# powei-lin/camera-intrinsic-calibration-rs

Measured on AMD Instinct MI355X. Metric: corner residual+Jacobian evals/sec; LM iters/sec to converge (EUCM, TUM-VI cam0), higher is better.
Workload: dtype f64

## Files before the change

camera_intrinsic_calibration_rs_amd/csrc/ccal_api.hip:

```cpp
#include <algorithm>
#include <cmath>
#include <cstdio>
#include <cstring>
#include <memory>
#include <new>

#include "ccal_call.hpp"
#include "ccal_normal.hpp"

using namespace ccal;

static void stream_synced(ccal_problem* p) {
    if (!p->nws) return;
    p->nws->tail_pending = false;
    if (p->nws->fws) p->nws->fws->tail_pending = false;
}

static void default_conventions(ccal_model_conventions* cv) {
    cv->kb4_small_radius = kDefaultKb4SmallRadius;
    cv->unproject_small_radius = kDefaultUnprojectSmallRadius;
    for (int i = 0; i < 5; ++i) cv->ocv5_order[i] = i;
    cv->reserved_ = 0;
    for (int m = 0; m < kNumModels; ++m)
        for (int i = 0; i < kMaxDist; ++i) { cv->dist_lo[m][i] = kDefaultDistLo[m][i]; cv->dist_hi[m][i] = kDefaultDistHi[m][i]; }
}
static_assert(sizeof(((ccal_model_conventions*)nullptr)->dist_lo) == sizeof(kDefaultDistLo), "conventions table shape");

extern "C" {

int ccal_get_model_conventions(const ccal_ctx* ctx, ccal_model_conventions* out) {
    if (!ctx || !out) return CCAL_ERR_INVALID_ARG;
    *out = ctx->conv;
    return CCAL_OK;
}
int ccal_set_model_conventions(ccal_ctx* ctx, const ccal_model_conventions* in) {
    if (!ctx) return CCAL_ERR_INVALID_ARG;
    if (!in) { default_conventions(&ctx->conv); return CCAL_OK; }
    if (!(in->kb4_small_radius >= 0.0) || !(in->unproject_small_radius >= 0.0)) return CCAL_ERR_INVALID_ARG;
    {
        int seen = 0;
        for (int i = 0; i < 5; ++i) { if (in->ocv5_order[i] < 0 || in->ocv5_order[i] > 4) return CCAL_ERR_INVALID_ARG; seen |= 1 << in->ocv5_order[i]; }
        if (seen != 31) return CCAL_ERR_INVALID_ARG;
    }
    for (int m = 0; m < kNumModels; ++m)
        for (int i = 0; i < model_np(m) - 4; ++i) if (!(in->dist_lo[m][i] <= in->dist_hi[m][i])) return CCAL_ERR_INVALID_ARG;
    ctx->conv = *in;
    return CCAL_OK;
}

const char* ccal_version(void) { return "ccal-mi355x 0.3.0 (gfx950)"; }
int ccal_model_num_params(int model) { return (model >= 0 && model < kNumModels) ? model_np(model) : model == CCAL_MODEL_EUCMT ? 8 : -1; }

int ccal_ctx_create(int device_id, void* hip_stream, ccal_ctx** out) {
    if (!out) return CCAL_ERR_INVALID_ARG;
    *out = nullptr;
    int n = 0;
    if (hipGetDeviceCount(&n) != hipSuccess || n <= 0) { (void)hipGetLastError(); note_create_error("ccal_ctx_create: no HIP device"); return CCAL_ERR_HIP; }
    if (device_id < 0 || device_id >= n) { note_create_error("ccal_ctx_create: device " + std::to_string(device_id) + " of " + std::to_string(n)); return CCAL_ERR_HIP; }
    ccal_ctx* c = new (std::nothrow) ccal_ctx();
    if (!c) return CCAL_ERR_NO_MEMORY;
    default_conventions(&c->conv);
    c->device = device_id;
    if (hipSetDevice(device_id) != hipSuccess) { delete c; note_create_error("ccal_ctx_create: hipSetDevice failed"); return CCAL_ERR_HIP; }
    if (hip_stream) { c->stream = (hipStream_t)hip_stream; c->own_stream = false; }
    else {
        if (hipStreamCreateWithFlags(&c->stream, hipStreamNonBlocking) != hipSuccess) { delete c; note_create_error("ccal_ctx_create: hipStreamCreate failed"); return CCAL_ERR_HIP; }
        c->own_stream = true;
    }
    *out = c;
    return CCAL_OK;
}
static void ctx_free(ccal_ctx* ctx) {
    ctx_worker_destroy(ctx);
    (void)hipSetDevice(ctx->device);
    ctx_release(ctx, ctx->d_batch_tab, false); ctx_release(ctx, ctx->h_batch_tab, true);
    ctx_cache_clear(ctx);
    if (!ctx->pinned.empty()) {
        (void)hipSetDevice(ctx->device);
        if (ctx->stream) (void)hipStreamSynchronize(ctx->stream);
        for (auto& pr : ctx->pinned) (void)hipHostUnregister(pr.first);
        (void)hipGetLastError();
        ctx->pinned.clear();
    }
    if (ctx->own_stream && ctx->stream) { (void)hipSetDevice(ctx->device); (void)hipStreamDestroy(ctx->stream); }
    delete ctx;
}
}
namespace ccal {
void ctx_unref(ccal_ctx* ctx) {
    if (--ctx->n_problems == 0 && ctx->destroy_requested) ctx_free(ctx);
}
}
extern "C" {
void ccal_ctx_destroy(ccal_ctx* ctx) {
    if (!ctx) return;
    if (ctx->n_problems > 0) { ctx->destroy_requested = true; return; }
    ctx_free(ctx);
}
const char* ccal_last_error(const ccal_ctx* ctx) { return ctx ? ctx->err.c_str() : "null context"; }
int ccal_sync(ccal_ctx* ctx) {
    if (!ctx) return CCAL_ERR_INVALID_ARG;
    HIP_TRY(ctx, hipSetDevice(ctx->device));
    HIP_TRY(ctx, hipStreamSynchronize(ctx->stream));
    return CCAL_OK;
}

int ccal_pin_buffer(ccal_ctx* ctx, void* host_ptr, size_t bytes) {
    if (!ctx || !host_ptr || !bytes) return CCAL_ERR_INVALID_ARG;
    CCAL_API_TRY
    HIP_TRY(ctx, hipSetDevice(ctx->device));
    for (auto& pr : ctx->pinned) if (pr.first == host_ptr) return fail(ctx, CCAL_ERR_INVALID_ARG, "ccal_pin_buffer: this address is pinned already");
    if (pinned_device_ptr(host_ptr, bytes)) return CCAL_OK;
    ctx->pinned.reserve(ctx->pinned.size() + 1);
    const hipError_t e = hipHostRegister(host_ptr, bytes, hipHostRegisterMapped | hipHostRegisterPortable);
    if (e != hipSuccess) { (void)hipGetLastError(); return fail(ctx, CCAL_ERR_HIP, (std::string("ccal_pin_buffer: hipHostRegister: ") + hipGetErrorString(e)).c_str()); }
    ctx->pinned.emplace_back(host_ptr, bytes);
    return CCAL_OK;
    CCAL_API_CATCH(ctx)
}
int ccal_unpin_buffer(ccal_ctx* ctx, void* host_ptr) {
    if (!ctx || !host_ptr) return CCAL_ERR_INVALID_ARG;
    CCAL_API_TRY
    for (size_t i = 0; i < ctx->pinned.size(); ++i) {
        if (ctx->pinned[i].first != host_ptr) continue;
        HIP_TRY(ctx, hipSetDevice(ctx->device));
        HIP_TRY(ctx, hipStreamSynchronize(ctx->stream));
        ctx->pinned.erase(ctx->pinned.begin() + (ptrdiff_t)i);
        HIP_TRY(ctx, hipHostUnregister(host_ptr));
        return CCAL_OK;
    }
    return CCAL_OK;
    CCAL_API_CATCH(ctx)
}

int ccal_set_defaults(ccal_solver_opts* o) {
    if (!o) return CCAL_ERR_INVALID_ARG;
    o->method = CCAL_METHOD_GN; o->max_iterations = 100;
    o->min_abs_error_decrease = 1e-5; o->min_rel_error_decrease = 1e-5; o->min_error = 1e-10;
    o->lm_initial_radius = 1e4; o->lm_min_diagonal = 1e-6; o->lm_max_diagonal = 1e32;
    o->verbose = 0; o->timeout_s = 0;
    o->error_metric = CCAL_ERROR_SQUARED_NORM; o->reserved_ = 0;
    return CCAL_OK;
}

int ccal_problem_create(ccal_ctx* ctx, const ccal_problem_desc* d, ccal_problem** out) {
    if (!ctx || !d || !out) return CCAL_ERR_INVALID_ARG;
    *out = nullptr;
    CCAL_API_TRY
    if (d->n_cams < 1 || d->n_cams > CCAL_MAX_CAMS || d->n_slots < 0 || d->n_obs < 0 || !d->model ||
        (d->n_obs > 0 && (!d->obs_cam || !d->obs_slot || !d->obs_offsets)))
        return fail(ctx, CCAL_ERR_INVALID_ARG, "bad problem description");
    HIP_TRY(ctx, hipSetDevice(ctx->device));
    struct Destroy { void operator()(ccal_problem* q) const { ccal_problem_destroy(q); } };
    std::unique_ptr<ccal_problem, Destroy> hold(new ccal_problem());
    ccal_problem* p = hold.get();
    p->ctx = ctx; p->n_cams = d->n_cams; p->n_slots = d->n_slots; p->n_obs = d->n_obs;
    p->one_focal = d->xy_same_focal != 0; p->huber_delta = d->huber_delta;
    p->cams.resize(d->n_cams);
    int K = 0;
    for (int c = 0; c < d->n_cams; ++c) {
        CamLayout& cl = p->cams[c];
        cl.model = d->model[c];
        if (cl.model == CCAL_MODEL_EUCMT) return fail(ctx, CCAL_ERR_UNSUPPORTED, "EUCMT is a parameter container in this build (its projection is only in the absent camera-intrinsic-model crate)");
        if (cl.model < 0 || cl.model >= kNumModels) return fail(ctx, CCAL_ERR_INVALID_ARG, "unknown camera model");
        cl.P = model_np(cl.model); cl.Peff = cl.P - (p->one_focal ? 1 : 0);
        cl.D = cl.Peff + (c == 0 ? 6 : 12);
        cl.col_theta = K; K += cl.Peff;
        if (c > 0) { cl.col_extr = K; K += 6; }
        cl.width = d->width ? d->width[c] : 0.0; cl.height = d->height ? d->height[c] : 0.0;
    }
    if (K >= CCAL_KMAX) return fail(ctx, CCAL_ERR_INVALID_ARG, "reduced system too large");
    p->K = K;
    if (d->n_obs > 0) {
        p->h_obs_off.assign(d->obs_offsets, d->obs_offsets + d->n_obs + 1);
        p->h_obs_cam.assign(d->obs_cam, d->obs_cam + d->n_obs);
        p->h_obs_slot.assign(d->obs_slot, d->obs_slot + d->n_obs);
    } else {
        p->h_obs_off.assign(1, 0);
    }
    p->h_joff.resize(d->n_obs + 1);
    std::vector<uint8_t> seen((size_t)d->n_cams * (size_t)std::max(d->n_slots, 1), 0);
    int64_t j = 0;
    for (int o = 0; o < d->n_obs; ++o) {
        const int cam = p->h_obs_cam[o], slot = p->h_obs_slot[o];
        const int64_t n = p->h_obs_off[o + 1] - p->h_obs_off[o];
        if (cam < 0 || cam >= d->n_cams || slot < 0 || slot >= d->n_slots || n < 0 || p->h_obs_off[0] != 0)
            return fail(ctx, CCAL_ERR_INVALID_ARG, "bad observation frame table");
        uint8_t& sn = seen[(size_t)cam * d->n_slots + slot];
        if (sn) return fail(ctx, CCAL_ERR_INVALID_ARG, "two observation frames for the same (camera, slot)");
        sn = 1;
        p->h_joff[o] = j; j += n * 2 * p->cams[cam].D;
        p->cams[cam].obs.push_back(o);
    }
    p->h_joff[d->n_obs] = j; p->j_len = j;
    p->slot_ident = d->n_slots == d->n_obs;
    for (int o = 0; o < d->n_obs && p->slot_ident; ++o) p->slot_ident = p->h_obs_slot[o] == o;
    p->n_corners = p->h_obs_off[d->n_obs];
    if (p->n_corners >= ((int64_t)1 << 30)) return fail(ctx, CCAL_ERR_INVALID_ARG, "more than 2^30 - 1 corners in one problem: shard the frames (ccal_multi_problem_create)");
    const size_t nc = (size_t)p->n_corners;
    if (nc && (!d->p3d_x || !d->p3d_y || !d->p3d_z || !d->p2d_u || !d->p2d_v)) return fail(ctx, CCAL_ERR_INVALID_ARG, "null corner arrays");
    {
        uint32_t any = 0;
        for (size_t i = 0; i < nc; ++i) { uint32_t b; std::memcpy(&b, d->p3d_z + i, sizeof b); any |= b & 0x7fffffffu; }
        p->has_nonplanar = any != 0;
    }
    std::vector<int32_t> bin_tab;
    if (d->n_cams == 1 && d->n_obs > 0) {
        std::vector<int32_t> order;
        const int m0 = p->cams[0].model;
        p->gram_bins = gram2_bin_plan(p->h_obs_off.data(), d->n_obs, m0 == kUCM || m0 == kEUCM, &order);
        if (p->gram_bins.n_bins > 0) {
            bin_tab.assign((size_t)d->n_obs * 4 + 4, 0);
            for (int i = 0; i < d->n_obs; ++i) {
                const int o = order[(size_t)i];
                bin_tab[4 * (size_t)i] = o; bin_tab[4 * (size_t)i + 1] = (int32_t)p->h_obs_off[o];
                bin_tab[4 * (size_t)i + 2] = (int32_t)(p->h_obs_off[o + 1] - p->h_obs_off[o]); bin_tab[4 * (size_t)i + 3] = p->h_obs_slot[o];
            }
        }
    }
    size_t cam_obs[CCAL_MAX_CAMS];
    for (int c = 0; c < d->n_cams; ++c) cam_obs[c] = p->cams[c].obs.size();
    const ProblemLayout l((size_t)p->n_corners, (size_t)d->n_obs, (size_t)d->n_slots, d->n_cams, cam_obs, bin_tab.size());
    const size_t total = l.plan.total;
    HIP_TRY(ctx, ctx_dev_alloc(ctx, (void**)&p->d_block, total));
    char* h_pack = nullptr;
    struct PackGuard { ccal_ctx* c; char*& p; ~PackGuard() { if (p) { (void)hipStreamSynchronize(c->stream); ccal::ctx_release(c, p, true); } } } pack_guard{ ctx, h_pack };
    if (total <= ((size_t)8 << 20)) HIP_TRY(ctx, ctx_host_alloc(ctx, (void**)&h_pack, total));
    if (!h_pack) HIP_TRY(ctx, hipMemsetAsync(p->d_block, 0, total, ctx->stream));
    {
        const Bound dev{ p->d_block }, img{ h_pack };
        auto put = [&](auto** dst, auto slice, const auto* src, size_t n) -> hipError_t {
            *dst = dev.at(slice);
            const size_t nb = src ? n * sizeof(*src) : 0;
            if (!h_pack) return nb ? hipMemcpyAsync(*dst, src, nb, hipMemcpyHostToDevice, ctx->stream) : hipSuccess;
            if (nb) std::memcpy(img.at(slice), src, nb);
            if (slice.bytes) std::memset((char*)img.at(slice) + nb, 0, slice.bytes - nb);
            return hipSuccess;
        };
        HIP_TRY(ctx, put(&p->d_x, l.x, d->p3d_x, nc)); HIP_TRY(ctx, put(&p->d_y, l.y, d->p3d_y, nc)); HIP_TRY(ctx, put(&p->d_z, l.z, d->p3d_z, nc));
        HIP_TRY(ctx, put(&p->d_u, l.u, d->p2d_u, nc)); HIP_TRY(ctx, put(&p->d_v, l.v, d->p2d_v, nc));
        HIP_TRY(ctx, put(&p->d_obs_off, l.obs_off, p->h_obs_off.data(), p->h_obs_off.size()));
        HIP_TRY(ctx, put(&p->d_joff, l.joff, p->h_joff.data(), p->h_joff.size()));
        HIP_TRY(ctx, put(&p->d_obs_cam, l.obs_cam, p->h_obs_cam.data(), p->h_obs_cam.size()));
        HIP_TRY(ctx, put(&p->d_obs_slot, l.obs_slot, p->h_obs_slot.data(), p->h_obs_slot.size()));
        for (int c = 0; c < d->n_cams; ++c) HIP_TRY(ctx, put(&p->cams[c].d_obs, l.cam_obs[c], p->cams[c].obs.data(), p->cams[c].obs.size()));
        HIP_TRY(ctx, put(&p->d_bin_tab, l.bin_tab, bin_tab.data(), bin_tab.size()));
        p->d_intr = dev.at(l.intr); p->d_poses = dev.at(l.poses); p->d_extr = dev.at(l.extr);
        p->d_intr_c = dev.at(l.intr_c); p->d_poses_c = dev.at(l.poses_c); p->d_extr_c = dev.at(l.extr_c);
        if (h_pack) {
            HIP_TRY(ctx, hipMemcpyAsync(p->d_block, h_pack, l.uploaded, hipMemcpyHostToDevice, ctx->stream));
            HIP_TRY(ctx, hipMemsetAsync(p->d_block + l.uploaded, 0, total - l.uploaded, ctx->stream));
        }
    }
    const size_t ni = (size_t)d->n_cams * CCAL_PMAX;
    p->lo.assign(ni, 0.0); p->hi.assign(ni, 0.0); p->has_bound.assign(ni, 0); p->fixed.assign(ni, 0);
    if (hipStreamSynchronize(ctx->stream) != hipSuccess) return fail(ctx, CCAL_ERR_HIP, "upload failed");
    p->counted = true;
    ctx->n_problems += 1;
    *out = hold.release();
    return CCAL_OK;
    CCAL_API_CATCH(ctx)
}

void ccal_problem_destroy(ccal_problem* p) {
    if (!p) return;
    if (p->nws && p->ctx && (p->nws->tail_pending || (p->nws->fws && p->nws->fws->tail_pending))) {
        (void)hipSetDevice(p->ctx->device);
        (void)hipDeviceSynchronize();
        p->nws->tail_pending = false;
        if (p->nws->fws) p->nws->fws->tail_pending = false;
    }
    ccal_ctx* ctx = p->ctx;
    if (ctx && (p->d_block || p->nws)) {
        (void)hipSetDevice(ctx->device);
        if (ctx->own_stream && ctx->stream) (void)hipStreamSynchronize(ctx->stream); else (void)hipDeviceSynchronize();
        (void)hipGetLastError();
    }
    void* ptrs[] = { p->d_block, p->d_r, p->d_J, p->d_err, p->d_scratch };
    for (void* q : ptrs) if (q) ctx_release(ctx, q, false);
    normal_ws_destroy(p);
    const bool counted = p->counted;
    delete p;
    if (ctx && counted && --ctx->n_problems == 0 && ctx->destroy_requested) ctx_free(ctx);
}

int64_t ccal_num_corners(const ccal_problem* p) { return p ? p->n_corners : -1; }
int ccal_reduced_dim(const ccal_problem* p) { return p ? p->K : -1; }
int ccal_block_dim(const ccal_problem* p, int cam) { return (p && cam >= 0 && cam < p->n_cams) ? p->cams[cam].D : -1; }
int ccal_eff_num_params(const ccal_problem* p, int cam) { return (p && cam >= 0 && cam < p->n_cams) ? p->cams[cam].Peff : -1; }
int64_t ccal_jacobian_len(const ccal_problem* p) { return p ? p->j_len : -1; }

static bool idx_ok(const ccal_problem* p, int cam, int idx) {
    return p && cam >= 0 && cam < p->n_cams && idx >= 0 && idx < p->cams[cam].Peff;
}
int ccal_set_bounds(ccal_problem* p, int cam, int idx, double lo, double hi) {
    if (!idx_ok(p, cam, idx) || !(lo <= hi)) return CCAL_ERR_INVALID_ARG;
    p->lo[cam * CCAL_PMAX + idx] = lo; p->hi[cam * CCAL_PMAX + idx] = hi; p->has_bound[cam * CCAL_PMAX + idx] = 1;
    return CCAL_OK;
}
int ccal_clear_bounds(ccal_problem* p, int cam, int idx) {
    if (!idx_ok(p, cam, idx)) return CCAL_ERR_INVALID_ARG;
    p->has_bound[cam * CCAL_PMAX + idx] = 0; return CCAL_OK;
}
int ccal_fix_param(ccal_problem* p, int cam, int idx) {
    if (!idx_ok(p, cam, idx)) return CCAL_ERR_INVALID_ARG;
    p->fixed[cam * CCAL_PMAX + idx] = 1; return CCAL_OK;
}
int ccal_unfix_param(ccal_problem* p, int cam, int idx) {
    if (!idx_ok(p, cam, idx)) return CCAL_ERR_INVALID_ARG;
    p->fixed[cam * CCAL_PMAX + idx] = 0; return CCAL_OK;
}

int ccal_apply_reference_bounds(ccal_problem* p) {
    if (!p) return CCAL_ERR_INVALID_ARG;
    const int shift = p->one_focal ? 1 : 0;
    const ccal_model_conventions& cv = p->ctx->conv;
    for (int c = 0; c < p->n_cams; ++c) {
        const CamLayout& cl = p->cams[c];
        ccal_set_bounds(p, c, 0, 0.0, 10000.0);
        ccal_set_bounds(p, c, 1 - shift, 0.0, 10000.0);
        ccal_set_bounds(p, c, 2 - shift, 0.0, cl.width);
        ccal_set_bounds(p, c, 3 - shift, 0.0, cl.height);
        for (int i = 4; i < cl.P; ++i) {
            const int at = cl.model == kOCV5 ? 4 + cv.ocv5_order[i - 4] : i;
            ccal_set_bounds(p, c, at - shift, cv.dist_lo[cl.model][i - 4], cv.dist_hi[cl.model][i - 4]);
        }
    }
    return CCAL_OK;
}
int ccal_disable_distortions(ccal_problem* p, int n_disabled, double* intr_io) {
    if (!p || n_disabled < 0) return CCAL_ERR_INVALID_ARG;
    const int shift = p->one_focal ? 1 : 0;
    for (int c = 0; c < p->n_cams; ++c) {
        for (int i = 0; i < n_disabled; ++i) {
            const int eff = p->cams[c].P - 1 - shift - i;
            if (eff < 0) return CCAL_ERR_INVALID_ARG;
            ccal_fix_param(p, c, eff);
            if (intr_io) intr_io[c * CCAL_PMAX + eff + shift] = 0.0;
        }
    }
    return CCAL_OK;
}
int ccal_set_allreduce(ccal_problem* p, ccal_allreduce_fn fn, void* user) {
    if (!p) return CCAL_ERR_INVALID_ARG;
    if (p->allreduce != fn || p->allreduce_user != user) { const int rc = drain_pending_groups(p); if (rc != CCAL_OK) return rc; }
    p->allreduce = fn; p->allreduce_user = user;
    return CCAL_OK;
}

int ccal_upload_params(ccal_problem* p, const double* intr, const double* poses, const double* extr) {
    if (!p) return CCAL_ERR_INVALID_ARG;
    ccal_ctx* ctx = p->ctx;
    HIP_TRY(ctx, hipSetDevice(ctx->device));
    if (intr) HIP_TRY(ctx, hipMemcpyAsync(p->d_intr, intr, sizeof(double) * p->n_cams * CCAL_PMAX, hipMemcpyHostToDevice, ctx->stream));
    if (poses && p->n_slots) HIP_TRY(ctx, hipMemcpyAsync(p->d_poses, poses, sizeof(double) * p->n_slots * 6, hipMemcpyHostToDevice, ctx->stream));
    if (extr) HIP_TRY(ctx, hipMemcpyAsync(p->d_extr, extr, sizeof(double) * p->n_cams * 6, hipMemcpyHostToDevice, ctx->stream));
    HIP_TRY(ctx, hipStreamSynchronize(ctx->stream));
    stream_synced(p);
    return CCAL_OK;
}
int ccal_download_params(ccal_problem* p, double* intr, double* poses, double* extr) {
    if (!p) return CCAL_ERR_INVALID_ARG;
    ccal_ctx* ctx = p->ctx;
    HIP_TRY(ctx, hipSetDevice(ctx->device));
    if (intr) HIP_TRY(ctx, hipMemcpyAsync(intr, p->d_intr, sizeof(double) * p->n_cams * CCAL_PMAX, hipMemcpyDeviceToHost, ctx->stream));
    if (poses && p->n_slots) HIP_TRY(ctx, hipMemcpyAsync(poses, p->d_poses, sizeof(double) * p->n_slots * 6, hipMemcpyDeviceToHost, ctx->stream));
    if (extr) HIP_TRY(ctx, hipMemcpyAsync(extr, p->d_extr, sizeof(double) * p->n_cams * 6, hipMemcpyDeviceToHost, ctx->stream));
    HIP_TRY(ctx, hipStreamSynchronize(ctx->stream));
    stream_synced(p);
    if (intr && p->one_focal) for (int c = 0; c < p->n_cams; ++c) intr[c * CCAL_PMAX + 1] = intr[c * CCAL_PMAX];
    return CCAL_OK;
}

static KArgs make_args(const ccal_problem* p, int cam) {
    KArgs a = {};
    a.x = p->d_x; a.y = p->d_y; a.z = p->d_z; a.u = p->d_u; a.v = p->d_v;
    a.obs_off = p->d_obs_off; a.obs_slot = p->d_obs_slot; a.joff = p->d_joff;
    a.list = p->cams[cam].d_obs; a.n_list = (int32_t)p->cams[cam].obs.size(); a.cam = cam;
    a.intr = p->d_intr; a.poses = p->d_poses; a.extr = p->d_extr;
    a.huber_delta = p->huber_delta; a.rt = model_rt(p->ctx);
    return a;
}

int ccal_eval_dev(ccal_problem* p, int apply_loss, double* r_dev, double* J_dev) {
    if (!p || !r_dev || !J_dev) return CCAL_ERR_INVALID_ARG;
    ccal_ctx* ctx = p->ctx;
    HIP_TRY(ctx, hipSetDevice(ctx->device));
    for (int c = 0; c < p->n_cams; ++c) {
        KArgs a = make_args(p, c);
        a.apply_loss = apply_loss; a.r_out = r_dev; a.J_out = J_dev;
        HIP_TRY(ctx, launch_eval(p, c, a, ctx->stream));
    }
    return CCAL_OK;
}

int ccal_eval(ccal_problem* p, const double* intr, const double* poses, const double* extr,
              int apply_loss, double* r_out, double* J_out) {
    if (!p || !intr || (!poses && p->n_slots) || (!extr && p->n_cams > 1) || !r_out || !J_out) return CCAL_ERR_INVALID_ARG;
    ccal_ctx* ctx = p->ctx;
    int rc = ccal_upload_params(p, intr, poses, extr);
    if (rc != CCAL_OK) return rc;
    HIP_TRY(ctx, ctx_doubles(ctx, &p->d_r, (size_t)std::max<int64_t>(2 * p->n_corners, 2)));
    HIP_TRY(ctx, ctx_doubles(ctx, &p->d_J, (size_t)std::max<int64_t>(p->j_len, 2)));
    rc = ccal_eval_dev(p, apply_loss, p->d_r, p->d_J);
    if (rc != CCAL_OK) return rc;
    if (p->n_corners) {
        HIP_TRY(ctx, hipMemcpyAsync(r_out, p->d_r, sizeof(double) * 2 * p->n_corners, hipMemcpyDeviceToHost, ctx->stream));
        HIP_TRY(ctx, hipMemcpyAsync(J_out, p->d_J, sizeof(double) * p->j_len, hipMemcpyDeviceToHost, ctx->stream));
    }
    HIP_TRY(ctx, hipStreamSynchronize(ctx->stream));
    return CCAL_OK;
}

}
namespace ccal {
int reprojection_errors_dev(ccal_problem* p, const double* intr, const double* poses, const double* extr, int only_cam) {
    ccal_ctx* ctx = p->ctx;
    int rc = ccal_upload_params(p, intr, poses, extr);
    if (rc != CCAL_OK) return rc;
    HIP_TRY(ctx, ctx_doubles(ctx, &p->d_err, (size_t)std::max<int64_t>(p->n_corners, 1)));
    for (int c = 0; c < p->n_cams; ++c) {
        if (only_cam >= 0 && c != only_cam) continue;
        KArgs a = make_args(p, c);
        a.err_out = p->d_err;
        HIP_TRY(ctx, launch_reproj_err(p, c, a, ctx->stream));
    }
    return CCAL_OK;
}
}
extern "C" {

int ccal_reprojection_errors(ccal_problem* p, const double* intr, const double* poses, const double* extr, double* err_out) {
    if (!p || !intr || (!poses && p->n_slots) || (!extr && p->n_cams > 1) || !err_out) return CCAL_ERR_INVALID_ARG;
    ccal_ctx* ctx = p->ctx;
    int rc = reprojection_errors_dev(p, intr, poses, extr);
    if (rc != CCAL_OK) return rc;
    if (p->n_corners) HIP_TRY(ctx, hipMemcpyAsync(err_out, p->d_err, sizeof(double) * p->n_corners, hipMemcpyDeviceToHost, ctx->stream));
    HIP_TRY(ctx, hipStreamSynchronize(ctx->stream));
    return CCAL_OK;
}

int ccal_init_poses(ccal_problem* p, const double* intr, int min_points, double* poses_obs, int32_t* n_used) {
    if (!p || !intr || !poses_obs || !n_used) return CCAL_ERR_INVALID_ARG;
    ccal_ctx* ctx = p->ctx;
    int rc = ccal_upload_params(p, intr, nullptr, nullptr);
    if (rc != CCAL_OK) return rc;
    const size_t no = (size_t)std::max(p->n_obs, 1);
    const PoseScratch l((size_t)p->n_obs);
    HIP_TRY(ctx, ensure_scratch(p, l.plan));
    double* d_po = Bound{ p->d_scratch }.at(l.poses);
    int32_t* d_va = Bound{ p->d_scratch }.at(l.counts);
    hipError_t e = hipMemsetAsync(d_va, 0, no * sizeof(int32_t), ctx->stream);
    for (int c = 0; c < p->n_cams && e == hipSuccess; ++c) e = launch_pose_init(p, c, p->d_intr, d_po, d_va, min_points, ctx->stream);
    if (e == hipSuccess && p->n_obs) {
        e = hipMemcpyAsync(poses_obs, d_po, (size_t)p->n_obs * 6 * sizeof(double), hipMemcpyDeviceToHost, ctx->stream);
        if (e == hipSuccess) e = hipMemcpyAsync(n_used, d_va, (size_t)p->n_obs * sizeof(int32_t), hipMemcpyDeviceToHost, ctx->stream);
    }
    if (e == hipSuccess) e = hipStreamSynchronize(ctx->stream);
    if (e != hipSuccess) { ctx->err = std::string("ccal_init_poses: ") + hipGetErrorString(e); return CCAL_ERR_HIP; }
    return CCAL_OK;
}

int ccal_validation(ccal_problem* p, int cam, const double* intr, const double* poses, const double* extr,
                    double* avg_99, double* median) {
    if (!p || cam < 0 || cam >= p->n_cams || !avg_99 || !median || !intr || (!poses && p->n_slots) || (!extr && p->n_cams > 1)) return CCAL_ERR_INVALID_ARG;
    ccal_ctx* ctx = p->ctx;
    if (p->cams[cam].obs.empty()) return fail(ctx, CCAL_ERR_INVALID_ARG, "camera has no observations");
    int rc = reprojection_errors_dev(p, intr, poses, extr, cam);
    if (rc != CCAL_OK) return rc;
    HIP_TRY(ctx, validation_stats_device(p, cam, p->d_err, avg_99, median, ctx->stream));
    return CCAL_OK;
}

}
```

camera_intrinsic_calibration_rs_amd/csrc/ccal_kernels_eval.hip:

```cpp
#include "ccal_device.hpp"
#include "ccal_gram_plan.hpp"
#include "ccal_internal.hpp"

#include <algorithm>
#include <type_traits>

namespace ccal {

__device__ __forceinline__ void wave_lds_sync() {
    __builtin_amdgcn_fence(__ATOMIC_RELEASE, "wavefront");
    __builtin_amdgcn_wave_barrier();
    __builtin_amdgcn_fence(__ATOMIC_ACQUIRE, "wavefront");
}

#ifndef CCAL_EVAL_WPB
#define CCAL_EVAL_WPB 2
#endif
#ifndef CCAL_EVAL_NT
#define CCAL_EVAL_NT 1
#endif
#ifndef CCAL_EVAL_NTR
#define CCAL_EVAL_NTR 0
#endif
#ifndef CCAL_EVAL_PREFETCH
#define CCAL_EVAL_PREFETCH -1
#endif
#ifndef CCAL_EVAL_PERSIST
#define CCAL_EVAL_PERSIST 0
#endif

constexpr int eval_tile_stride(int D) { return 2 * D + ((D & 1) ? 4 : 2); }
template <bool OTHER> constexpr int fc_doubles() { return OTHER ? FC_SIZE : FC_N0P; }

template <int MODEL, bool OF, bool OTHER, bool PF, bool AL>
__global__ __launch_bounds__(64 * CCAL_EVAL_WPB) void k_eval(const KArgs a) {
    constexpr int D = block_dim(MODEL, OF, OTHER);
    constexpr int TW = 2 * D;
    constexpr int TS = eval_tile_stride(D);
    constexpr int FCN = fc_doubles<OTHER>();
    constexpr int WS = FCN + 64 * TS;
    extern __shared__ double smem[];
    const int wave = threadIdx.x >> 6, lane = threadIdx.x & 63;
    double* fc = smem + wave * WS;
    double* tile = fc + FCN;
    const int wstride = CCAL_EVAL_PERSIST > 0 ? (int)gridDim.x * CCAL_EVAL_WPB : a.n_list;
    for (int widx = blockIdx.x * CCAL_EVAL_WPB + wave; widx < a.n_list; widx += wstride) {
    const int o = __builtin_amdgcn_readfirstlane(a.list[widx]);
    const int slot = __builtin_amdgcn_readfirstlane(a.obs_slot[o]);
    const int64_t start = a.obs_off[o];
    const int n = (int)(a.obs_off[o + 1] - start);
    const double* th_g = a.intr + a.cam * CCAL_PMAX;
    double th[th_len<MODEL>()];
    load_theta<MODEL, OF>(th_g, a.rt, th);

    float pX = 0.f, pY = 0.f, pZ = 0.f, pU = 0.f, pV = 0.f;
    if constexpr (PF) {
        if (n > 0) {
            const int64_t g0 = start + (lane < n ? lane : 0);
            pX = a.x[g0]; pY = a.y[g0]; pZ = a.z[g0]; pU = a.u[g0]; pV = a.v[g0];
        }
    }
    {
        double pose[6], ex[6];
#pragma unroll
        for (int i = 0; i < 6; ++i) pose[i] = a.poses[(int64_t)slot * 6 + i];
        if constexpr (OTHER) {
#pragma unroll
            for (int i = 0; i < 6; ++i) ex[i] = a.extr[a.cam * 6 + i];
        }
        double fcr[OTHER ? FC_SIZE : FC_N0];
        frame_setup<OTHER>(pose, ex, fcr);
        if (lane == 0) {
#pragma unroll
            for (int i = 0; i < (OTHER ? FC_SIZE : FC_N0); ++i) fc[i] = fcr[i];
        }
    }
    wave_lds_sync();

    const int64_t jbase = a.joff[o];
    auto pass = [&](auto full_tag, const int base) {
        constexpr bool FULL = decltype(full_tag)::value;
        const int c = base + lane;
        const bool valid = FULL || c < n;
        const int64_t g = start + (valid ? c : 0);
        double X, Y, Z, uo, vo;
        if constexpr (PF) {
            X = pX; Y = pY; Z = pZ; uo = pU; vo = pV;
            if (base + 64 < n) {
                const int cn = base + 64 + lane;
                const int64_t gn = start + (cn < n ? cn : 0);
                pX = a.x[gn]; pY = a.y[gn]; pZ = a.z[gn]; pU = a.u[gn]; pV = a.v[gn];
            }
        } else {
            X = a.x[g]; Y = a.y[g]; Z = a.z[g]; uo = a.u[g]; vo = a.v[g];
        }
        double ru, rv, J[TW];
        double* Ju = J;
        double* Jv = J + D;
#if defined(CCAL_EVAL_DIAG) && CCAL_EVAL_DIAG == 2
        ru = X + uo; rv = Y + vo;
#pragma unroll
        for (int i = 0; i < D; ++i) { Ju[i] = X * (double)(i + 1) + fc[0]; Jv[i] = Z * (double)(i + 1) + vo; }
#else
        corner_block<MODEL, OF, OTHER>(th, fc, X, Y, Z, uo, vo, ru, rv, Ju, Jv);
#endif
        if constexpr (AL) {
            const double sw = huber_sqrt_weight(ru * ru + rv * rv, a.huber_delta);
            ru *= sw; rv *= sw;
#pragma unroll
            for (int i = 0; i < D; ++i) { Ju[i] *= sw; Jv[i] *= sw; }
        }
#if CCAL_EVAL_NTR
        if (valid) { __builtin_nontemporal_store(ru, a.r_out + 2 * g); __builtin_nontemporal_store(rv, a.r_out + 2 * g + 1); }
#else
        if (valid) *reinterpret_cast<double2*>(a.r_out + 2 * g) = make_double2(ru, rv);
#endif
        double* row = tile + lane * TS;
#pragma unroll
        for (int i = 0; i < D; ++i) *reinterpret_cast<double2*>(row + 2 * i) = make_double2(J[2 * i], J[2 * i + 1]);
        if constexpr (MODEL == kOCV5) {
            if (a.rt.ocv5_perm != kOcv5IdentityPerm) {
                constexpr int D0 = OF ? 3 : 4;
#pragma unroll
                for (int i = 0; i < 5; ++i) {
                    const int at = D0 + ocv5_pos(a.rt.ocv5_perm, i);
                    row[at] = J[D0 + i]; row[D + at] = J[D + D0 + i];
                }
            }
        }
        wave_lds_sync();
        double* dst = a.J_out + jbase + (int64_t)base * TW;
        auto put = [&](const int e) {
            const int cr = e / TW;
            const int k = e - cr * TW;
            const double2 val = *reinterpret_cast<const double2*>(tile + cr * TS + k);
#if defined(CCAL_EVAL_DIAG) && CCAL_EVAL_DIAG == 1
            if (e != lane * 2 || val.x != 12345.678) return;
#endif
#if CCAL_EVAL_NT
            __builtin_nontemporal_store(val.x, dst + e);
            __builtin_nontemporal_store(val.y, dst + e + 1);
#else
            *reinterpret_cast<double2*>(dst + e) = val;
#endif
        };
        if constexpr (FULL) {
#pragma unroll
            for (int it = 0; it < TW / 2; ++it) put(lane * 2 + 128 * it);
        } else {
            const int tot = (n - base) * TW;
            for (int e = lane * 2; e < tot; e += 128) put(e);
        }
        wave_lds_sync();
    };
    const int n_full = n & ~63;
    for (int base = 0; base < n_full; base += 64) pass(std::true_type{}, base);
    if (n_full < n) pass(std::false_type{}, n_full);
    }
}

template <int MODEL, bool OF, bool OTHER>
__global__ __launch_bounds__(256) void k_reproj_err(const KArgs a) {
    constexpr int FCN = fc_doubles<OTHER>();
    __shared__ double smem[WAVES_PER_BLOCK * FCN];
    const int wave = threadIdx.x >> 6, lane = threadIdx.x & 63;
    const int widx = blockIdx.x * WAVES_PER_BLOCK + wave;
    if (widx >= a.n_list) return;
    double* fc = smem + wave * FCN;
    const int o = __builtin_amdgcn_readfirstlane(a.list[widx]);
    const int slot = __builtin_amdgcn_readfirstlane(a.obs_slot[o]);
    const int64_t start = a.obs_off[o];
    const int n = (int)(a.obs_off[o + 1] - start);
    const double* th_g = a.intr + a.cam * CCAL_PMAX;
    double th[th_len<MODEL>()];
    load_theta<MODEL, OF>(th_g, a.rt, th);
    {
        double pose[6], ex[6];
#pragma unroll
        for (int i = 0; i < 6; ++i) pose[i] = a.poses[(int64_t)slot * 6 + i];
        if constexpr (OTHER) {
#pragma unroll
            for (int i = 0; i < 6; ++i) ex[i] = a.extr[a.cam * 6 + i];
        }
        double fcr[OTHER ? FC_SIZE : FC_N0];
        frame_setup<OTHER>(pose, ex, fcr);
        if (lane == 0) {
#pragma unroll
            for (int i = 0; i < 12; ++i) fc[i] = fcr[i];
        }
    }
    wave_lds_sync();
    for (int c = lane; c < n; c += 64) {
        const int64_t g = start + c;
        double px, py, pz, u, v;
        transform_point(fc, a.x[g], a.y[g], a.z[g], px, py, pz);
        project_uv<MODEL>(th, px, py, pz, u, v);
        const double du = u - (double)a.u[g], dv = v - (double)a.v[g];
        a.err_out[g] = sqrt(du * du + dv * dv);
    }
}

template <int MODEL, bool OF, bool OTHER, bool PF, bool AL>
static hipError_t launch_eval_pf(const KArgs& a, hipStream_t s) {
    constexpr int D = block_dim(MODEL, OF, OTHER);
    constexpr int WS = fc_doubles<OTHER>() + 64 * eval_tile_stride(D);
    const size_t lds = sizeof(double) * WS * CCAL_EVAL_WPB;
    int blocks = (a.n_list + CCAL_EVAL_WPB - 1) / CCAL_EVAL_WPB;
    if (blocks == 0) return hipSuccess;
    if (CCAL_EVAL_PERSIST > 0) blocks = std::min(blocks, 256 * CCAL_EVAL_PERSIST);
    static DynLdsGuard lds_guard;
    if (hipError_t e = ensure_dyn_lds(reinterpret_cast<const void*>(&k_eval<MODEL, OF, OTHER, PF, AL>), lds, lds_guard); e != hipSuccess) return e;
    hipLaunchKernelGGL((k_eval<MODEL, OF, OTHER, PF, AL>), dim3(blocks), dim3(64 * CCAL_EVAL_WPB), lds, s, a);
    return hipGetLastError();
}
#ifndef CCAL_EVAL_PF_MIN_D
#define CCAL_EVAL_PF_MIN_D 99
#endif
template <int MODEL, bool OF, bool OTHER> constexpr bool eval_prefetch_always() { return block_dim(MODEL, OF, OTHER) >= CCAL_EVAL_PF_MIN_D; }
template <int MODEL, bool OF, bool OTHER>
static hipError_t launch_eval_t(const KArgs& a, bool big_inputs, hipStream_t s) {
    const bool pf = CCAL_EVAL_PREFETCH < 0 ? (big_inputs || eval_prefetch_always<MODEL, OF, OTHER>()) : CCAL_EVAL_PREFETCH != 0;
    if (a.apply_loss) return pf ? launch_eval_pf<MODEL, OF, OTHER, true, true>(a, s) : launch_eval_pf<MODEL, OF, OTHER, false, true>(a, s);
    return pf ? launch_eval_pf<MODEL, OF, OTHER, true, false>(a, s) : launch_eval_pf<MODEL, OF, OTHER, false, false>(a, s);
}
template <int MODEL, bool OF, bool OTHER>
static hipError_t launch_err_t(const KArgs& a, hipStream_t s) {
    const int blocks = (a.n_list + WAVES_PER_BLOCK - 1) / WAVES_PER_BLOCK;
    if (blocks == 0) return hipSuccess;
    hipLaunchKernelGGL((k_reproj_err<MODEL, OF, OTHER>), dim3(blocks), dim3(256), 0, s, a);
    return hipGetLastError();
}

hipError_t launch_eval(const ccal_problem* p, int cam, const KArgs& a, hipStream_t s) {
    const bool big_inputs = p->n_corners * 20 > (int64_t)120 << 20;
    return dispatch_model_focal_other(p->cams[cam].model, p->one_focal, cam > 0, hipErrorInvalidValue, [&](auto m, auto of, auto other) {
        return launch_eval_t<decltype(m)::value, decltype(of)::value, decltype(other)::value>(a, big_inputs, s);
    });
}
hipError_t launch_reproj_err(const ccal_problem* p, int cam, const KArgs& a, hipStream_t s) {
    return dispatch_model_focal_other(p->cams[cam].model, p->one_focal, cam > 0, hipErrorInvalidValue, [&](auto m, auto of, auto other) {
        return launch_err_t<decltype(m)::value, decltype(of)::value, decltype(other)::value>(a, s);
    });
}

}
```

Baseline: 27.56 billion.

## Add frame-per-workgroup eval kernel with 3 waves sharing frame constants

Adds k_eval_fw, which assigns one observation (frame) to a 3-wave workgroup. The waves share the frame constants in LDS and stride over corners in steps of 192 with prefetch, instead of one wave walking all corners of a frame. It is selected by default when inputs are not big and the frame count is at most 10000, and the pass body is moved into a shared device function. Separately, large uploads now go through a 4 MB pinned staging buffer with a synchronize after each chunk, and asm barriers are added around the Huber weighting.

```diff
diff --git a/camera_intrinsic_calibration_rs_amd/csrc/ccal_api.hip b/camera_intrinsic_calibration_rs_amd/csrc/ccal_api.hip
--- a/camera_intrinsic_calibration_rs_amd/csrc/ccal_api.hip
+++ b/camera_intrinsic_calibration_rs_amd/csrc/ccal_api.hip
@@ -226,13 +226,28 @@
     char* h_pack = nullptr;
     struct PackGuard { ccal_ctx* c; char*& p; ~PackGuard() { if (p) { (void)hipStreamSynchronize(c->stream); ccal::ctx_release(c, p, true); } } } pack_guard{ ctx, h_pack };
     if (total <= ((size_t)8 << 20)) HIP_TRY(ctx, ctx_host_alloc(ctx, (void**)&h_pack, total));
-    if (!h_pack) HIP_TRY(ctx, hipMemsetAsync(p->d_block, 0, total, ctx->stream));
+    constexpr size_t kStageBytes = (size_t)4 << 20;
+    char* h_stage = nullptr;
+    PackGuard stage_guard{ ctx, h_stage };
+    if (!h_pack) {
+        HIP_TRY(ctx, ctx_host_alloc(ctx, (void**)&h_stage, kStageBytes));
+        HIP_TRY(ctx, hipMemsetAsync(p->d_block, 0, total, ctx->stream));
+    }
     {
         const Bound dev{ p->d_block }, img{ h_pack };
         auto put = [&](auto** dst, auto slice, const auto* src, size_t n) -> hipError_t {
             *dst = dev.at(slice);
             const size_t nb = src ? n * sizeof(*src) : 0;
-            if (!h_pack) return nb ? hipMemcpyAsync(*dst, src, nb, hipMemcpyHostToDevice, ctx->stream) : hipSuccess;
+            if (!h_pack) {
+                for (size_t off = 0; off < nb; off += kStageBytes) {
+                    const size_t m = std::min(kStageBytes, nb - off);
+                    std::memcpy(h_stage, reinterpret_cast<const char*>(src) + off, m);
+                    hipError_t e = hipMemcpyAsync(reinterpret_cast<char*>(*dst) + off, h_stage, m, hipMemcpyHostToDevice, ctx->stream);
+                    if (e == hipSuccess) e = hipStreamSynchronize(ctx->stream);
+                    if (e != hipSuccess) return e;
+                }
+                return hipSuccess;
+            }
             if (nb) std::memcpy(img.at(slice), src, nb);
             if (slice.bytes) std::memset((char*)img.at(slice) + nb, 0, slice.bytes - nb);
             return hipSuccess;
diff --git a/camera_intrinsic_calibration_rs_amd/csrc/ccal_kernels_eval.hip b/camera_intrinsic_calibration_rs_amd/csrc/ccal_kernels_eval.hip
--- a/camera_intrinsic_calibration_rs_amd/csrc/ccal_kernels_eval.hip
+++ b/camera_intrinsic_calibration_rs_amd/csrc/ccal_kernels_eval.hip
@@ -1,4 +1,5 @@
 #include "ccal_device.hpp"
+#include "ccal_devopt.hpp"
 #include "ccal_gram_plan.hpp"
 #include "ccal_internal.hpp"
 
@@ -32,10 +33,116 @@
 constexpr int eval_tile_stride(int D) { return 2 * D + ((D & 1) ? 4 : 2); }
 template <bool OTHER> constexpr int fc_doubles() { return OTHER ? FC_SIZE : FC_N0P; }
 
+
+__device__ __forceinline__ void eval_request_rows(const KArgs& a, const int64_t start, const int n, const int base, const int lane,
+                                                  float& pX, float& pY, float& pZ, float& pU, float& pV) {
+    if (base < n) {
+        const int c = base + lane;
+        const int64_t g = start + (c < n ? c : 0);
+        pX = a.x[g]; pY = a.y[g]; pZ = a.z[g]; pU = a.u[g]; pV = a.v[g];
+    }
+}
+
+template <bool OTHER>
+__device__ __forceinline__ void eval_frame_constants(const KArgs& a, const int slot, const int lane, double* fc) {
+    double pose[6], ex[6];
+#pragma unroll
+    for (int i = 0; i < 6; ++i) pose[i] = a.poses[(int64_t)slot * 6 + i];
+    if constexpr (OTHER) {
+#pragma unroll
+        for (int i = 0; i < 6; ++i) ex[i] = a.extr[a.cam * 6 + i];
+    }
+    double fcr[OTHER ? FC_SIZE : FC_N0];
+    frame_setup<OTHER>(pose, ex, fcr);
+    if (lane == 0) {
+#pragma unroll
+        for (int i = 0; i < (OTHER ? FC_SIZE : FC_N0); ++i) fc[i] = fcr[i];
+    }
+}
+
+template <int MODEL, bool OF, bool OTHER, bool PF, bool AL, bool FULL, int STEP>
+__device__ __forceinline__ void eval_pass(const KArgs& a, const double* th, const double* fc, double* tile, const int lane,
+                                          const int64_t start, const int n, const int64_t jbase, const int base,
+                                          float& pX, float& pY, float& pZ, float& pU, float& pV) {
+    constexpr int D = block_dim(MODEL, OF, OTHER);
+    constexpr int TW = 2 * D;
+    constexpr int TS = eval_tile_stride(D);
+    const int c = base + lane;
+    const bool valid = FULL || c < n;
+    const int64_t g = start + (valid ? c : 0);
+    double X, Y, Z, uo, vo;
+    if constexpr (PF) {
+        X = pX; Y = pY; Z = pZ; uo = pU; vo = pV;
+        eval_request_rows(a, start, n, base + STEP, lane, pX, pY, pZ, pU, pV);
+    } else {
+        X = a.x[g]; Y = a.y[g]; Z = a.z[g]; uo = a.u[g]; vo = a.v[g];
+    }
+    double ru, rv, J[TW];
+    double* Ju = J;
+    double* Jv = J + D;
+#if defined(CCAL_EVAL_DIAG) && CCAL_EVAL_DIAG == 2
+    ru = X + uo; rv = Y + vo;
+#pragma unroll
+    for (int i = 0; i < D; ++i) { Ju[i] = X * (double)(i + 1) + fc[0]; Jv[i] = Z * (double)(i + 1) + vo; }
+#else
+    corner_block<MODEL, OF, OTHER>(th, fc, X, Y, Z, uo, vo, ru, rv, Ju, Jv);
+#endif
+    if constexpr (AL) {
+        asm volatile("" : "+v"(ru), "+v"(rv));
+#pragma unroll
+        for (int i = 0; i < D; ++i) asm volatile("" : "+v"(Ju[i]), "+v"(Jv[i]));
+        const double sw = huber_sqrt_weight(ru * ru + rv * rv, a.huber_delta);
+        ru *= sw; rv *= sw;
+#pragma unroll
+        for (int i = 0; i < D; ++i) { Ju[i] *= sw; Jv[i] *= sw; }
+    }
+#if CCAL_EVAL_NTR
+    if (valid) { __builtin_nontemporal_store(ru, a.r_out + 2 * g); __builtin_nontemporal_store(rv, a.r_out + 2 * g + 1); }
+#else
+    if (valid) *reinterpret_cast<double2*>(a.r_out + 2 * g) = make_double2(ru, rv);
+#endif
+    double* row = tile + lane * TS;
+#pragma unroll
+    for (int i = 0; i < D; ++i) *reinterpret_cast<double2*>(row + 2 * i) = make_double2(J[2 * i], J[2 * i + 1]);
+    if constexpr (MODEL == kOCV5) {
+        if (a.rt.ocv5_perm != kOcv5IdentityPerm) {
+            constexpr int D0 = OF ? 3 : 4;
+#pragma unroll
+            for (int i = 0; i < 5; ++i) {
+                const int at = D0 + ocv5_pos(a.rt.ocv5_perm, i);
+                row[at] = J[D0 + i]; row[D + at] = J[D + D0 + i];
+            }
+        }
+    }
+    wave_lds_sync();
+    double* dst = a.J_out + jbase + (int64_t)base * TW;
+    auto put = [&](const int e) {
+        const int cr = e / TW;
+        const int k = e - cr * TW;
+        const double2 val = *reinterpret_cast<const double2*>(tile + cr * TS + k);
+#if defined(CCAL_EVAL_DIAG) && CCAL_EVAL_DIAG == 1
+        if (e != lane * 2 || val.x != 12345.678) return;
+#endif
+#if CCAL_EVAL_NT
+        __builtin_nontemporal_store(val.x, dst + e);
+        __builtin_nontemporal_store(val.y, dst + e + 1);
+#else
+        *reinterpret_cast<double2*>(dst + e) = val;
+#endif
+    };
+    if constexpr (FULL) {
+#pragma unroll
+        for (int it = 0; it < TW / 2; ++it) put(lane * 2 + 128 * it);
+    } else {
+        const int tot = (n - base) * TW;
+        for (int e = lane * 2; e < tot; e += 128) put(e);
+    }
+    wave_lds_sync();
+}
+
 template <int MODEL, bool OF, bool OTHER, bool PF, bool AL>
 __global__ __launch_bounds__(64 * CCAL_EVAL_WPB) void k_eval(const KArgs a) {
     constexpr int D = block_dim(MODEL, OF, OTHER);
-    constexpr int TW = 2 * D;
     constexpr int TS = eval_tile_stride(D);
     constexpr int FCN = fc_doubles<OTHER>();
     constexpr int WS = FCN + 64 * TS;
@@ -54,12 +161,7 @@
     load_theta<MODEL, OF>(th_g, a.rt, th);
 
     float pX = 0.f, pY = 0.f, pZ = 0.f, pU = 0.f, pV = 0.f;
-    if constexpr (PF) {
-        if (n > 0) {
-            const int64_t g0 = start + (lane < n ? lane : 0);
-            pX = a.x[g0]; pY = a.y[g0]; pZ = a.z[g0]; pU = a.u[g0]; pV = a.v[g0];
-        }
-    }
+    if constexpr (PF) eval_request_rows(a, start, n, 0, lane, pX, pY, pZ, pU, pV);
     {
         double pose[6], ex[6];
 #pragma unroll
@@ -78,85 +180,39 @@
     wave_lds_sync();
 
     const int64_t jbase = a.joff[o];
-    auto pass = [&](auto full_tag, const int base) {
-        constexpr bool FULL = decltype(full_tag)::value;
-        const int c = base + lane;
-        const bool valid = FULL || c < n;
-        const int64_t g = start + (valid ? c : 0);
-        double X, Y, Z, uo, vo;
-        if constexpr (PF) {
-            X = pX; Y = pY; Z = pZ; uo = pU; vo = pV;
-            if (base + 64 < n) {
-                const int cn = base + 64 + lane;
-                const int64_t gn = start + (cn < n ? cn : 0);
-                pX = a.x[gn]; pY = a.y[gn]; pZ = a.z[gn]; pU = a.u[gn]; pV = a.v[gn];
-            }
-        } else {
-            X = a.x[g]; Y = a.y[g]; Z = a.z[g]; uo = a.u[g]; vo = a.v[g];
-        }
-        double ru, rv, J[TW];
-        double* Ju = J;
-        double* Jv = J + D;
-#if defined(CCAL_EVAL_DIAG) && CCAL_EVAL_DIAG == 2
-        ru = X + uo; rv = Y + vo;
-#pragma unroll
-        for (int i = 0; i < D; ++i) { Ju[i] = X * (double)(i + 1) + fc[0]; Jv[i] = Z * (double)(i + 1) + vo; }
-#else
-        corner_block<MODEL, OF, OTHER>(th, fc, X, Y, Z, uo, vo, ru, rv, Ju, Jv);
-#endif
-        if constexpr (AL) {
-            const double sw = huber_sqrt_weight(ru * ru + rv * rv, a.huber_delta);
-            ru *= sw; rv *= sw;
-#pragma unroll
-            for (int i = 0; i < D; ++i) { Ju[i] *= sw; Jv[i] *= sw; }
-        }
-#if CCAL_EVAL_NTR
-        if (valid) { __builtin_nontemporal_store(ru, a.r_out + 2 * g); __builtin_nontemporal_store(rv, a.r_out + 2 * g + 1); }
-#else
-        if (valid) *reinterpret_cast<double2*>(a.r_out + 2 * g) = make_double2(ru, rv);
-#endif
-        double* row = tile + lane * TS;
-#pragma unroll
-        for (int i = 0; i < D; ++i) *reinterpret_cast<double2*>(row + 2 * i) = make_double2(J[2 * i], J[2 * i + 1]);
-        if constexpr (MODEL == kOCV5) {
-            if (a.rt.ocv5_perm != kOcv5IdentityPerm) {
-                constexpr int D0 = OF ? 3 : 4;
-#pragma unroll
-                for (int i = 0; i < 5; ++i) {
-                    const int at = D0 + ocv5_pos(a.rt.ocv5_perm, i);
-                    row[at] = J[D0 + i]; row[D + at] = J[D + D0 + i];
-                }
-            }
-        }
-        wave_lds_sync();
-        double* dst = a.J_out + jbase + (int64_t)base * TW;
-        auto put = [&](const int e) {
-            const int cr = e / TW;
-            const int k = e - cr * TW;
-            const double2 val = *reinterpret_cast<const double2*>(tile + cr * TS + k);
-#if defined(CCAL_EVAL_DIAG) && CCAL_EVAL_DIAG == 1
-            if (e != lane * 2 || val.x != 12345.678) return;
-#endif
-#if CCAL_EVAL_NT
-            __builtin_nontemporal_store(val.x, dst + e);
-            __builtin_nontemporal_store(val.y, dst + e + 1);
-#else
-            *reinterpret_cast<double2*>(dst + e) = val;
-#endif
-        };
-        if constexpr (FULL) {
-#pragma unroll
-            for (int it = 0; it < TW / 2; ++it) put(lane * 2 + 128 * it);
-        } else {
-            const int tot = (n - base) * TW;
-            for (int e = lane * 2; e < tot; e += 128) put(e);
-        }
-        wave_lds_sync();
-    };
     const int n_full = n & ~63;
-    for (int base = 0; base < n_full; base += 64) pass(std::true_type{}, base);
-    if (n_full < n) pass(std::false_type{}, n_full);
-    }
+    for (int base = 0; base < n_full; base += 64)
+        eval_pass<MODEL, OF, OTHER, PF, AL, true, 64>(a, th, fc, tile, lane, start, n, jbase, base, pX, pY, pZ, pU, pV);
+    if (n_full < n) eval_pass<MODEL, OF, OTHER, PF, AL, false, 64>(a, th, fc, tile, lane, start, n, jbase, n_full, pX, pY, pZ, pU, pV);
+    }
+}
+
+constexpr int kEvalFwWaves = 3;
+template <int MODEL, bool OF, bool OTHER, bool AL>
+__global__ __launch_bounds__(64 * kEvalFwWaves) void k_eval_fw(const KArgs a) {
+    constexpr int D = block_dim(MODEL, OF, OTHER);
+    constexpr int TS = eval_tile_stride(D);
+    constexpr int FCN = fc_doubles<OTHER>();
+    constexpr int STEP = 64 * kEvalFwWaves;
+    extern __shared__ double smem[];
+    const int wave = __builtin_amdgcn_readfirstlane(threadIdx.x >> 6), lane = threadIdx.x & 63;
+    double* fc = smem;
+    double* tile = smem + FCN + wave * (64 * TS);
+    const int o = __builtin_amdgcn_readfirstlane(a.list[blockIdx.x]);
+    const int64_t start = a.obs_off[o];
+    const int n = (int)(a.obs_off[o + 1] - start);
+    const double* th_g = a.intr + a.cam * CCAL_PMAX;
+    double th[th_len<MODEL>()];
+    load_theta<MODEL, OF>(th_g, a.rt, th);
+    float pX = 0.f, pY = 0.f, pZ = 0.f, pU = 0.f, pV = 0.f;
+    eval_request_rows(a, start, n, 64 * wave, lane, pX, pY, pZ, pU, pV);
+    if (wave == 0) eval_frame_constants<OTHER>(a, __builtin_amdgcn_readfirstlane(a.obs_slot[o]), lane, fc);
+    __syncthreads();
+    const int64_t jbase = a.joff[o];
+    int base = 64 * wave;
+    for (; base + 64 <= n; base += STEP)
+        eval_pass<MODEL, OF, OTHER, true, AL, true, STEP>(a, th, fc, tile, lane, start, n, jbase, base, pX, pY, pZ, pU, pV);
+    if (base < n) eval_pass<MODEL, OF, OTHER, true, AL, false, STEP>(a, th, fc, tile, lane, start, n, jbase, base, pX, pY, pZ, pU, pV);
 }
 
 template <int MODEL, bool OF, bool OTHER>
@@ -217,8 +273,36 @@
 #define CCAL_EVAL_PF_MIN_D 99
 #endif
 template <int MODEL, bool OF, bool OTHER> constexpr bool eval_prefetch_always() { return block_dim(MODEL, OF, OTHER) >= CCAL_EVAL_PF_MIN_D; }
+
+#ifndef CCAL_EVAL_FW_MAX_FRAMES
+#define CCAL_EVAL_FW_MAX_FRAMES 10000
+#endif
+template <int MODEL, bool OF, bool OTHER> constexpr size_t eval_fw_lds_bytes() {
+    return sizeof(double) * (fc_doubles<OTHER>() + kEvalFwWaves * 64 * eval_tile_stride(block_dim(MODEL, OF, OTHER)));
+}
+constexpr bool eval_frame_form(int n_list, bool big_inputs) { return !big_inputs && n_list <= CCAL_EVAL_FW_MAX_FRAMES; }
+static_assert(eval_fw_lds_bytes<kEUCM, false, false>() == 40112 && eval_fw_lds_bytes<kEUCM, false, true>() <= 64 * 1024 &&
+              eval_fw_lds_bytes<kOCV5, false, true>() <= 160 * 1024, "k_eval_fw: a workgroup's LDS");
+static_assert(eval_frame_form(1, false) && eval_frame_form(625, false) && eval_frame_form(CCAL_EVAL_FW_MAX_FRAMES, false) &&
+              !eval_frame_form(CCAL_EVAL_FW_MAX_FRAMES + 1, false) && !eval_frame_form(625, true), "k_eval_fw: the selection rule");
+static int eval_form_forced() {
+    static const int v = [] { const char* e = dev_env("CCAL_EVAL_FORM"); return !e ? -1 : e[0] == 'f' ? 1 : e[0] == 'p' ? 0 : -1; }();
+    return v;
+}
+template <int MODEL, bool OF, bool OTHER, bool AL>
+static hipError_t launch_eval_fw(const KArgs& a, hipStream_t s) {
+    constexpr size_t lds = eval_fw_lds_bytes<MODEL, OF, OTHER>();
+    if (a.n_list == 0) return hipSuccess;
+    static DynLdsGuard lds_guard;
+    if (hipError_t e = ensure_dyn_lds(reinterpret_cast<const void*>(&k_eval_fw<MODEL, OF, OTHER, AL>), lds, lds_guard); e != hipSuccess) return e;
+    hipLaunchKernelGGL((k_eval_fw<MODEL, OF, OTHER, AL>), dim3(a.n_list), dim3(64 * kEvalFwWaves), lds, s, a);
+    return hipGetLastError();
+}
 template <int MODEL, bool OF, bool OTHER>
 static hipError_t launch_eval_t(const KArgs& a, bool big_inputs, hipStream_t s) {
+    const int forced = eval_form_forced();
+    if (forced < 0 ? eval_frame_form(a.n_list, big_inputs) : forced == 1)
+        return a.apply_loss ? launch_eval_fw<MODEL, OF, OTHER, true>(a, s) : launch_eval_fw<MODEL, OF, OTHER, false>(a, s);
     const bool pf = CCAL_EVAL_PREFETCH < 0 ? (big_inputs || eval_prefetch_always<MODEL, OF, OTHER>()) : CCAL_EVAL_PREFETCH != 0;
     if (a.apply_loss) return pf ? launch_eval_pf<MODEL, OF, OTHER, true, true>(a, s) : launch_eval_pf<MODEL, OF, OTHER, false, true>(a, s);
     return pf ? launch_eval_pf<MODEL, OF, OTHER, true, false>(a, s) : launch_eval_pf<MODEL, OF, OTHER, false, false>(a, s);
```

New measurement: 29.46 billion (median of 6 runs). 1.07x the previous value.
